# JackAILab/ConsistentID

Hardware: AMD Instinct MI355X
Metric: 512x512 SD1.5 images/sec/node @50 DDIM steps (higher is better)
Workload: dtype f16; 1 GPU; sd15 ConsistentID 512x512, 50 DDIM steps, batch 4/GPU (global 4), CFG batch 8, LoRA rank 128 merged, start_merge_step 30, hipGraph on; global_batch=4, parallelism=dp1 (images sharded, no in-step collective)

## Files before the change

### consistentid_amd/csrc/gemm.hip

```cpp
#include "xattn_core.h"
#include "gemm_args.h"
#include "../../include/cid.h"
#include <stdlib.h>

#ifndef CID_HALO_STAGGER
#define CID_HALO_STAGGER 1
#endif
#ifdef CID_CONV_TRACE
__device__ unsigned long long g_conv_trace[2 * 4096];
#define CONV_STAMP(k) do { if (tr_on) tr_ts[k] = __builtin_readcyclecounter(); } while (0)
#define CONV_FLUSH() do { if (tr_on && lane == 0 && tr_n + 8 <= 4096) { for (int q_ = 0; q_ < 8; ++q_) g_conv_trace[tr_slot * 4096 + tr_n + q_] = tr_ts[q_]; } tr_n += 8; } while (0)
#else
#define CONV_STAMP(k) do { } while (0)
#define CONV_FLUSH() do { } while (0)
#endif
#if defined(CID_GEMM_ABLATION)
#define CID_ABL(bit) ((a.ablate & (bit)) != 0)
#else
#define CID_ABL(bit) false
#endif

namespace {
using cidg::GemmArgs;
using cidg::wait_vmcnt;
// ... 936 lines not shown
                          : launch_one_ln<TM, TN, WM, WN, false, false, false, 3>(a, ncols, s);
    }
    return a.ln_s ? launch_one_ln<TM, TN, WM, WN, VMODE, true>(a, ncols, s) : launch_one_ln<TM, TN, WM, WN, VMODE, false>(a, ncols, s);
}

template <int TM, int TN, int WM, int WN, int ATT_D>
int launch_att(GemmArgs a, hipStream_t s) {
    a.n_begin = 0; a.n_end = a.N;
    return a.ln_s ? launch_one_ln<TM, TN, WM, WN, false, true, false, 2, ATT_D>(a, a.N, s)
                  : launch_one_ln<TM, TN, WM, WN, false, false, false, 2, ATT_D>(a, a.N, s);
}

template <int TM, int TN, int WM, int WN>
int launch_act(GemmArgs a, hipStream_t s) {
    a.n_begin = 0; a.n_end = a.N;
    return launch_one_ln<TM, TN, WM, WN, false, false, false, 2, 0, true>(a, a.N, s);
}

template <int TM, int TN, int WM, int WN>
int launch_halo(GemmArgs a, hipStream_t s) {
    constexpr int BM = 16 * TM * WM, BN = 16 * TN * WN, NW = WM * WN;
    constexpr int SMEM = 2 * (7 * NW * 1024) + 2 * (((BN / 8 + NW - 1) / NW) * NW * 1024);
    static_assert(SMEM <= 160 * 1024, "LDS budget");
    auto kern = igemm_halo_kernel<TM, TN, WM, WN>;
    static bool configured = false;
    if (!configured) {
        hipError_t herr = hipFuncSetAttribute((const void*)kern, hipFuncAttributeMaxDynamicSharedMemorySize, SMEM);
        if (herr != hipSuccess) {
            cid_set_error("cid_gemm_f16: cannot reserve %d bytes of LDS (%s)", SMEM, hipGetErrorString(herr));
            return -5;
        }
        configured = true;
    }
    a.n_begin = 0; a.n_end = a.N;
    dim3 grid((a.N + BN - 1) / BN, (a.M + BM - 1) / BM, a.splitk);
    a.xcd_pn = cidg::choose_xcd_pn((int)grid.x, (int)grid.y, 2.0 * a.N * a.ktot, (double)a.bytes_x1 + a.bytes_x2);
    hipLaunchKernelGGL(kern, grid, dim3(64 * NW), SMEM, s, a);
    if (a.splitk > 1) {
        const long items = (long)a.M * (a.N >> 2);
        const int g = (int)((items + 255) / 256 > 2048 ? 2048 : (items + 255) / 256);
        hipLaunchKernelGGL(splitk_epilogue_kernel, dim3(g), dim3(256), 0, s, a);
    }
    return 0;
}

template <int TM, int TN, int WM, int WN>
int launch(GemmArgs a, hipStream_t s) {
    const int n_plain = (a.mode == 2) ? a.n_vt0 : a.N;
    a.n_begin = 0; a.n_end = n_plain;
    int rc = launch_one<TM, TN, WM, WN, false>(a, n_plain, s);
    if (rc) return rc;
    if (a.splitk > 1) {
        const long items = (long)a.M * (a.N >> 2);
        const int grid = (int)((items + 255) / 256 > 2048 ? 2048 : (items + 255) / 256);
        hipLaunchKernelGGL(splitk_epilogue_kernel, dim3(grid), dim3(256), 0, s, a);
    }
    if (a.mode == 2 && a.N > a.n_vt0) {
        GemmArgs v = a;
        v.n_begin = a.n_vt0; v.n_end = a.N; v.splitk = 1;
        rc = launch_one<TM, TN, WM, WN, true>(v, a.N - a.n_vt0, s);
    }
    return rc;
}

}

int cidg::choose_xcd_pn(int gx, int gy, double w_bytes, double x_bytes) {
    static int on = -1;
    if (on < 0) { const char* e = getenv("CID_XCD_2D"); on = e ? atoi(e) : 1; }
    if (!on || ((long)gx * gy) % 8 != 0) return 0;
    int best = 0;
    double cost = 0.0;
    for (int pn = 1; pn <= 8; pn *= 2) {
        const int pm = 8 / pn;
        if (gx % pn != 0 || gy % pm != 0) continue;
        const double c = pm * w_bytes + pn * x_bytes;
        if (best == 0 || c < cost) { best = pn; cost = c; }
    }
    return best;
}

enum TileCfg { A256x160, B128x160, C64x160, G256x128, G128x128, O64x64, O128x32 };

static int plan_gemm(const cid_gemm_desc* d, GemmArgs& a, TileCfg& cfg, bool& halo, int& bm_out, bool& h32, bool& g32) {
    h32 = false;
    g32 = false;
    CID_CHECK_ARG(d && d->x1 && d->w && d->out, "cid_gemm_f16: null pointer");
    CID_CHECK_ARG(d->taps == 1 || d->taps == 9, "cid_gemm_f16: taps must be 1 or 9 (got %d)", d->taps);
    CID_CHECK_ARG(d->c1 > 0 && d->c1 % 32 == 0 && d->c2 >= 0 && d->c2 % 32 == 0 && (d->c1 + d->c2) % 64 == 0 &&
                  (d->c2 == 0 || d->c1 % 64 == 0),
                  "cid_gemm_f16: channel counts must be multiples of 64 (c1=%d c2=%d)", d->c1, d->c2);
    CID_CHECK_ARG(d->c2 == 0 || d->x2, "cid_gemm_f16: c2 > 0 needs x2");
    CID_CHECK_ARG(d->N > 0 && d->N % 32 == 0 && d->M > 0, "cid_gemm_f16: bad M/N (%d, %d)", d->M, d->N);
    CID_CHECK_ARG(d->mode >= 0 && d->mode <= 3, "cid_gemm_f16: bad mode %d", d->mode);
    CID_CHECK_ARG(d->ld1 % 8 == 0 && d->ldo % 8 == 0 && (d->c2 == 0 || d->ld2 % 8 == 0) && (!d->res || d->ldr % 8 == 0),
                  "cid_gemm_f16: row pitches (ld1, ld2, ldo, ldr) must keep 16-byte alignment");
    CID_CHECK_ARG((((uintptr_t)d->out | (uintptr_t)d->res | (uintptr_t)d->out2) & 15) == 0,
                  "cid_gemm_f16: out / out2 / res must be 16-byte aligned (rows are stored and the residual is read in 16-byte chunks)");
    CID_CHECK_ARG((d->ln_s == nullptr) == (d->ln_b == nullptr), "cid_gemm_f16: ln_s and ln_b come together");
    CID_CHECK_ARG(!d->ln_s || (d->taps == 1 && d->c2 == 0 && !d->bias && d->ln_eps > 0.f),
                  "cid_gemm_f16: the LayerNorm fold applies to one-source linears; the bias belongs in ln_b");
    a.x1 = (const half_t*)d->x1; a.x2 = (const half_t*)d->x2;
    a.c1 = d->c1; a.c2 = d->c2; a.ld1 = d->ld1; a.ld2 = d->ld2;
    a.w = (const half_t*)d->w; a.out = (half_t*)d->out; a.ldo = d->ldo;
    a.out2 = (half_t*)d->out2;
    CID_CHECK_ARG(!d->out2 || d->mode == 0, "cid_gemm_f16: out2 (a second destination) goes with the plain epilogue, mode 0");
    a.bias = (const half_t*)d->bias;
    a.rowbias = (const half_t*)d->rowbias; a.ld_rowbias = d->ld_rowbias;
    a.rows_per_sample = d->rows_per_sample > 0 ? d->rows_per_sample : 1;
    a.res = (const half_t*)d->res; a.ldr = d->ldr;
    a.M = d->M; a.N = d->N; a.taps = d->taps;
    a.Hi = d->Hi; a.Wi = d->Wi; a.Ho = d->Ho; a.Wo = d->Wo; a.stride = d->stride; a.up = d->up;
    a.mode = d->mode;
    a.vt = (half_t*)d->vt; a.n_vt0 = d->n_vt0; a.heads = d->heads; a.dhead = d->dhead;
    a.dvp = d->dvp; a.ntok = d->ntok;
    a.cslabs = (d->c1 + d->c2) / BK;
    a.ktot = d->taps * (d->c1 + d->c2);
    a.nslab = a.ktot / BK;
    a.splitk = 1;
    a.nloop = 1;
    a.nbuf = 2;
    a.xcd_pn = 0;
    a.att_kp = (const half_t*)d->att_kp; a.att_vp = (const half_t*)d->att_vp; a.att_kvrow = (const int*)d->att_kvrow;
    a.att_n_txt = d->att_n_txt; a.att_n_ip = d->att_n_ip; a.att_scale = d->att_ip_scale;
    a.att_krow = a.att_vrow = 0;
    a.ws = (float*)d->ws;
    a.ln_s = d->ln_s; a.ln_b = d->ln_b; a.ln_eps = d->ln_eps;
    a.gn_stats = d->gn_stats; a.gn_unit = d->N / 32;
    {
#if defined(CID_GEMM_ABLATION)
        static int ablate = -1;
        if (ablate < 0) { const char* e = getenv("CID_GEMM_ABLATE"); ablate = e ? atoi(e) : 0; }
        a.ablate = ablate;
#else
        a.ablate = 0;
#endif
    }
    {
        const long rows_in = (d->taps == 9) ? (long)(d->M / (d->Ho * d->Wo)) * d->Hi * d->Wi : (long)d->M;
        const long b1 = ((rows_in - 1) * d->ld1 + d->c1) * 2, b2 = d->c2 ? ((rows_in - 1) * d->ld2 + d->c2) * 2 : 0;
        const long bw = (long)d->N * a.ktot * 2;
        CID_CHECK_ARG(b1 < 0x7fffffffL && b2 < 0x7fffffffL && bw < 0x7fffffffL, "cid_gemm_f16: tensor exceeds 2 GiB");
        a.bytes_x1 = (unsigned)b1; a.bytes_x2 = (unsigned)b2; a.bytes_w = (unsigned)bw;
    }
    a.n_begin = 0; a.n_end = a.N;
    if (d->taps == 9) {
        CID_CHECK_ARG(d->Hi > 0 && d->Wi > 0 && d->Ho > 0 && d->Wo > 0 && (d->stride == 1 || d->stride == 2)
                      && (d->up == 0 || d->up == 1), "cid_gemm_f16: bad conv geometry");
        CID_CHECK_ARG(d->M % (d->Ho * d->Wo) == 0, "cid_gemm_f16: M is not batch * Ho * Wo");
    }
    CID_CHECK_ARG(d->pad_mode == 0 || d->pad_mode == 1, "cid_gemm_f16: bad pad_mode %d", d->pad_mode);
    CID_CHECK_ARG(d->pad_mode == 0 || (d->mode == 0 && d->taps == 9 && d->stride == 2 && d->up == 0 && d->Hi % 2 == 0 &&
                                       d->Wi % 2 == 0 && d->Ho == d->Hi / 2 && d->Wo == d->Wi / 2),
                  "cid_gemm_f16: pad_mode 1 needs mode 0, taps 9, stride 2, up 0, even Hi / Wi, Ho = Hi / 2 and Wo = Wi / 2 "
                  "(got mode %d taps %d stride %d up %d, %d x %d -> %d x %d)", d->mode, d->taps, d->stride, d->up, d->Hi, d->Wi,
                  d->Ho, d->Wo);
    a.tap0 = d->pad_mode == 1 ? 0 : -1;
    CID_CHECK_ARG(d->act == 0 || d->act == 1, "cid_gemm_f16: bad act %d", d->act);
    CID_CHECK_ARG(d->act == 0 || (d->mode == 0 && !d->gn_stats && !d->ws && !d->ln_s),
                  "cid_gemm_f16: act 1 needs mode 0 and no gn_stats / ws / ln_s (got mode %d)", d->mode);

    if (d->mode == 3) {
        CID_CHECK_ARG(d->att_kp && d->att_vp && d->att_kvrow, "cid_gemm_f16: mode 3 needs att_kp / att_vp / att_kvrow");
        CID_CHECK_ARG(d->taps == 1 && d->c2 == 0 && !d->bias && !d->rowbias && !d->res && !d->gn_stats,
                      "cid_gemm_f16: mode 3 is a plain projection (no bias / residual / statistics)");
        CID_CHECK_ARG(d->heads > 0 && d->dhead > 0 && d->N == d->heads * d->dhead && (d->dhead == 64 || d->dhead == 80 || d->dhead == 160),
                      "cid_gemm_f16: mode 3 needs N = heads * dhead with dhead in {64, 80, 160} (got %d x %d, N = %d)", d->heads, d->dhead, d->N);
        CID_CHECK_ARG(d->att_n_txt == 77 && d->att_n_ip == 4, "cid_gemm_f16: mode 3 is built for the reference's 77 + 4 context (got %d + %d)",
                      d->att_n_txt, d->att_n_ip);
        CID_CHECK_ARG(d->ntok > 0 && d->M % d->ntok == 0 && d->ntok % 64 == 0, "cid_gemm_f16: mode 3 needs ntok (tokens per sample, a multiple of 64)");
        const int qks = (d->dhead + 15) / 16, dvt = (d->dhead + 31) / 32;
        a.att_krow = (long)d->heads * 3 * qks * 512;
        a.att_vrow = (long)d->heads * dvt * 6 * 512;
        if (d->dhead == 64) { cfg = G128x128; bm_out = 128; CID_CHECK_ARG(d->N % 128 == 0 && d->ntok % 128 == 0, "cid_gemm_f16: mode 3, dhead 64: N and ntok multiples of 128"); }
        else {
            CID_CHECK_ARG(d->N % 160 == 0, "cid_gemm_f16: mode 3, dhead %d: N = %d is not a multiple of the 160-channel tile", d->dhead, d->N);
            if (d->ntok % 128 == 0 && (long)(d->M / 128) * (d->N / 160) >= 256) { cfg = B128x160; bm_out = 128; }
            else { cfg = C64x160; bm_out = 64; }
        }
        halo = false;
        return 0;
    }
    const int n_plain = (d->mode == 2) ? d->n_vt0 : d->N;
    const long target = 2048;
    auto waves = [&](int bm_, int bn_, int w) {
        return (long)((a.M + bm_ - 1) / bm_) * ((n_plain + bn_ - 1) / bn_) * w;
    };
    int bm = 0, bn = 0, nw = 0;
    bool small_tiles = (d->mode == 1) && (a.nslab <= 10 || waves(256, 128, 1) < 1024);
    if (d->mode == 1) {
        static int g_tile = -1;
        if (g_tile < 0) { const char* e = getenv("CID_GEGLU_TILE"); g_tile = e ? atoi(e) : 0; }
        if (g_tile == 1) small_tiles = false;
        if (g_tile == 2) small_tiles = true;
        if (d->N % 128 != 0) { cfg = O64x64; bm = 64; bn = 64; nw = 4; }
        else if (waves(256, 128, 8) >= target && !small_tiles) { cfg = G256x128; bm = 256; bn = 128; nw = 8; }
        else { cfg = G128x128; bm = 128; bn = 128; nw = 8; }
    } else if (n_plain % 160 == 0) {
        static int f_tile = -1, f_sk = -1;
        if (f_tile < 0) { const char* e = getenv("CID_GEMM_TILE"); f_tile = e ? atoi(e) : 0; }
        if (f_sk < 0) { const char* e = getenv("CID_GEMM_SK"); f_sk = e ? atoi(e) : 0; }
        const bool can_split = (d->mode == 0) && a.ws != nullptr && !a.ln_s;
        auto tiles = [&](int bm_) { return (long)((a.M + bm_ - 1) / bm_) * (n_plain / 160); };
        auto sk_for = [&](int bm_) {
            long t = tiles(bm_);
            int sk = (int)((256 + t - 1) / t);
            if (!can_split) sk = 1;
            if (sk > 16) sk = 16;
            while (sk > 1 && a.nslab / sk < 6) --sk;
            while (sk > 1 && (int64_t)sk * a.M * a.N * 4 > d->ws_bytes) --sk;
            return sk;
        };
        int pick = 0;
        bool nosplit = false;
        static int prefer128 = -1;
        if (prefer128 < 0) { const char* e = getenv("CID_GEMM_PREFER128"); prefer128 = e ? atoi(e) : 1; }
        if (f_tile) pick = f_tile;
        else if (d->taps == 1 && tiles(256) >= 256) {
            pick = (prefer128 || (d->mode == 2 && tiles(256) <= 512 && tiles(128) >= 512)) ? 2 : 1;
            nosplit = true;
        } else if (d->taps == 1 && tiles(128) >= 256 && (a.nslab <= 40 || prefer128)) { pick = 2; nosplit = true; }
        else if (d->taps == 1 && tiles(64) >= 256 && a.nslab <= 20) { pick = 3; nosplit = true; }
        else if (tiles(256) * sk_for(256) >= 256) pick = 1;
        else if (tiles(128) * sk_for(128) >= 256) pick = 2;
        else pick = 3;
        if (pick == 1)      { cfg = A256x160; bm = 256; bn = 160; nw = 8; }
// ... 9 lines not shown
    if (d->mode == 1) CID_CHECK_ARG(d->N % 64 == 0, "cid_gemm_f16: GEGLU needs N %% 64 == 0");
    if (d->mode == 1 && (cfg == G128x128 || cfg == G256x128) && d->taps == 1 && d->c2 == 0 && a.M % bm == 0) {
        static int f_nl = -1;
        if (f_nl < 0) { const char* e = getenv("CID_GEGLU_NLOOP"); f_nl = e ? atoi(e) : 0; }
        const int nt = d->N / bn;
        const long tiles = (long)(a.M / bm) * nt;
        int nl = f_nl > 0 ? f_nl : (int)(tiles / (cfg == G128x128 ? 512 : 256));
        if (nl > nt) nl = nt;
        while (nl > 1 && nt % nl != 0) --nl;
        if (nl > 1 && (long)nl * bn * a.ktot * 2 < 0x7fffffffL) a.nloop = nl;
    }
    if (d->mode == 1 && d->taps == 1 && d->c2 == 0 && !a.ln_s && d->N % 160 == 0 && a.M % 256 == 0 && a.cslabs >= 16) {
        static int f_g32 = -1;
        if (f_g32 < 0) { const char* e = getenv("CID_GEGLU_H32"); f_g32 = e ? atoi(e) : 1; }
        const int nt = d->N / 160;
        const long tiles = (long)(a.M / 256) * nt;
        int nl = (int)(tiles / 256);
        if (nl > nt) nl = nt;
        while (nl > 1 && nt % nl != 0) --nl;
        if (f_g32 && tiles >= 256 && nl >= 1 && (long)nl * 160 * a.ktot * 2 < 0x7fffffffL) {
            g32 = true;
            a.nloop = nl;
            bm = 256;
        }
    }
    if (d->mode == 2) {
        CID_CHECK_ARG(d->vt && d->ntok % 16 == 0 && d->M % d->ntok == 0 && d->n_vt0 % bn == 0 && d->dhead > 0
                      && d->heads > 0 && d->dvp >= d->dhead && (d->N - d->n_vt0) % 16 == 0,
                      "cid_gemm_f16: bad QKV/V^T description");
    }
    if (d->mode == 0 && a.ws && !a.ln_s && a.nslab >= 16 && n_plain % 160 != 0) {
        const long w = waves(bm, bn, nw);
        if (w < target) {
            int sk = (int)((target + w - 1) / w);
            if (sk > 8) sk = 8;
            while (sk > 1 && a.nslab / sk < 8) --sk;
            while (sk > 1 && (int64_t)sk * a.M * a.N * 4 > d->ws_bytes) --sk;
            a.splitk = sk;
        }
    }
    {
        static int f_nb = -1;
        if (f_nb < 0) { const char* e = getenv("CID_GEMM_NBUF"); f_nb = e ? atoi(e) : 0; }
        const bool legal = (cfg == A256x160 || cfg == B128x160 || cfg == C64x160) && d->mode != 1 && !d->act;
        const long wgs = (long)((a.M + bm - 1) / bm) * ((n_plain + bn - 1) / bn) * a.splitk;
        const bool want = cfg == A256x160 ? (a.nslab / a.splitk >= 4) : (wgs <= 256 && a.nslab / a.splitk >= 8);
        if (legal && (f_nb == 3 || (f_nb == 0 && want))) a.nbuf = 3;
    }
    static int no_halo = -1;
    if (no_halo < 0) { const char* e = getenv("CID_GEMM_NOHALO"); no_halo = e ? atoi(e) : 0; }
    halo = false;
    if (cfg == A256x160 && !no_halo && !d->act && d->mode == 0 && d->taps == 9 && d->stride == 1 && d->up == 0 && d->Wo == d->Wi &&
        d->Ho == d->Hi) {
        const int HW = d->Ho * d->Wo;
        const int seg = 256 < HW ? 256 : HW;
        const bool rows_ok = (seg % d->Wo == 0) && (HW % seg == 0) && (256 % seg == 0) && (d->M % 256 == 0);
        const int nh = (256 / seg) * (seg / d->Wo + 2) * (d->Wo + 2);
        if (rows_ok && nh <= 448) {
            halo = true;
            if (a.splitk > a.cslabs) a.splitk = a.cslabs;
        }
    }
    {
        static int no_h32 = -1;
        static int only256 = 0;
        if (no_h32 < 0) { const char* e = getenv("CID_CONV_H32"); no_h32 = (e && atoi(e) == 0) ? 1 : 0; only256 = (e && atoi(e) == 2) ? 1 : 0; }
        const int HW = d->taps == 9 ? d->Ho * d->Wo : 0;
        const bool shape_ok = !no_h32 && !d->act && d->mode == 0 && d->taps == 9 && d->stride == 1 && (d->up == 0 || d->up == 1) &&
                              d->Wo == (d->Wi << d->up) && d->Ho == (d->Hi << d->up) && d->N % 160 == 0 && HW >= 64 &&
                              (!d->rowbias || (a.rows_per_sample >= 64 && a.rows_per_sample % 64 == 0));
        for (int bm_try = 256; shape_ok && !h32 && bm_try >= (only256 ? 256 : 128); bm_try >>= 1) {
            const int seg = bm_try < HW ? bm_try : HW;
            if (seg % d->Wo != 0 || HW % seg != 0 || bm_try % seg != 0 || d->M % bm_try != 0) continue;
            if (d->up && (seg != bm_try || (seg / d->Wo) % 2 != 0)) continue;
            const int nh = (bm_try / seg) * (((seg / d->Wo) >> d->up) + 2) * ((d->Wo >> d->up) + 2);
            if (nh > 400) continue;
            const long tiles = (long)(d->M / bm_try) * (d->N / 160);
            if (tiles < 256 || (bm_try == 128 && a.cslabs > 10)) continue;
            h32 = true; halo = false;
            bm = bm_try;
            a.splitk = 1;
        }
    }
    bm_out = bm;
    if (a.gn_stats) {
        const bool ok = d->mode == 0 && a.splitk == 1 && (cfg == A256x160 || cfg == B128x160 || cfg == C64x160) &&
                        d->N % 32 == 0 && 80 % a.gn_unit == 0 && d->M % bm == 0;
        CID_CHECK_ARG(ok, "cid_gemm_f16: gn_stats requested for a launch that cannot emit them (ask cid_gemm_stats_rows first)");
    }
    return 0;
}

extern "C" int cid_gemm_stats_rows(const cid_gemm_desc* d) {
    if (!d) return 0;
    cid_gemm_desc q = *d;
    q.gn_stats = nullptr;
    GemmArgs a;
    TileCfg cfg;
    bool halo, h32, g32;
    int bm = 0;
    if (plan_gemm(&q, a, cfg, halo, bm, h32, g32) != 0) return 0;
    const int unit = d->N / 32;
    const bool ok = d->mode == 0 && d->act == 0 && a.splitk == 1 && (cfg == A256x160 || cfg == B128x160 || cfg == C64x160) &&
                    d->N % 32 == 0 && unit > 0 && 80 % unit == 0 && d->M % bm == 0;
    return ok ? bm : 0;
}

extern "C" int cid_gemm_f16(const cid_gemm_desc* d, cid_stream_t stream) {
    GemmArgs a;
    TileCfg cfg;
    bool halo, h32, g32;
    int bm = 0;
    int rc = plan_gemm(d, a, cfg, halo, bm, h32, g32);
    if (rc) return rc;
    hipStream_t s = (hipStream_t)stream;
    if (g32) {
        a.n_begin = 0; a.n_end = a.N;
        rc = cidg::launch_geglu_h32(a, s);
        if (rc) return rc;
        CID_CHECK_LAUNCH("cid_gemm_f16");
        return 0;
    }
    if (a.mode == 3) {
        if (cfg == G128x128) rc = launch_att<2, 4, 4, 2, 64>(a, s);
        else if (cfg == B128x160) rc = a.dhead == 80 ? launch_att<2, 5, 4, 2, 80>(a, s) : launch_att<2, 5, 4, 2, 160>(a, s);
        else rc = a.dhead == 80 ? launch_att<2, 5, 2, 2, 80>(a, s) : launch_att<2, 5, 2, 2, 160>(a, s);
        if (rc) return rc;
        CID_CHECK_LAUNCH("cid_gemm_f16");
        return 0;
    }
    if (d->act) {
        switch (cfg) {
            case A256x160: rc = launch_act<4, 5, 4, 2>(a, s); break;
            case B128x160: rc = launch_act<2, 5, 4, 2>(a, s); break;
            case C64x160:  rc = launch_act<2, 5, 2, 2>(a, s); break;
            case G256x128: rc = launch_act<4, 4, 4, 2>(a, s); break;
            case G128x128: rc = launch_act<2, 4, 4, 2>(a, s); break;
            case O64x64:   rc = launch_act<2, 2, 2, 2>(a, s); break;
            case O128x32:  rc = launch_act<2, 2, 4, 1>(a, s); break;
        }
        if (rc) return rc;
        CID_CHECK_LAUNCH("cid_gemm_f16");
        return 0;
    }
    if (h32) {
        a.n_begin = 0; a.n_end = a.N;
        rc = cidg::launch_conv_h32(a, bm, s);
        if (rc) return rc;
        CID_CHECK_LAUNCH("cid_gemm_f16");
        return 0;
    }
    if (halo) {
        rc = launch_halo<4, 5, 4, 2>(a, s);
        if (rc) return rc;
        CID_CHECK_LAUNCH("cid_gemm_f16");
        return 0;
    }
    switch (cfg) {
        case A256x160: rc = launch<4, 5, 4, 2>(a, s); break;
        case B128x160: rc = launch<2, 5, 4, 2>(a, s); break;
        case C64x160:  rc = launch<2, 5, 2, 2>(a, s); break;
        case G256x128: rc = launch<4, 4, 4, 2>(a, s); break;
        case G128x128: rc = launch<2, 4, 4, 2>(a, s); break;
        case O64x64:   rc = launch<2, 2, 2, 2>(a, s); break;
        case O128x32:  rc = launch<2, 2, 4, 1>(a, s); break;
    }
    if (rc) return rc;
    CID_CHECK_LAUNCH("cid_gemm_f16");
    return 0;
}
```

### consistentid_amd/csrc/gemm_args.h

```cpp
#pragma once
#include "common.h"

namespace cidg {

struct GemmArgs {
    const half_t* x1; const half_t* x2;
    int c1, c2, ld1, ld2;
    const half_t* w;
    half_t* out; int ldo;
    half_t* out2;
    const half_t* bias;
    const half_t* rowbias; int ld_rowbias; int rows_per_sample;
    const half_t* res; int ldr;
    int M, N, taps;
    int Hi, Wi, Ho, Wo, stride, up;
    int mode;
    half_t* vt; int n_vt0, heads, dhead, dvp, ntok;
    int n_begin, n_end;
    int ktot;
    int nslab;
    int cslabs;
    int splitk;
    int nloop;
    int nbuf;
    const half_t* att_kp; const half_t* att_vp; const int* att_kvrow;
    long att_krow, att_vrow;
    int att_n_txt, att_n_ip;
    float att_scale;
    unsigned bytes_x1, bytes_x2, bytes_w;
    float* ws;
    const float* ln_s;
    const float* ln_b;
    float ln_eps;
    float* gn_stats;
    int gn_unit;
    int ablate;
    int xcd_pn;
    int tap0;
};

CID_DEVINL void xcd_tile(const GemmArgs& a, int& nb, int& mb) {
    const int gx = gridDim.x, gy = gridDim.y;
    int bid = blockIdx.y * gx + blockIdx.x;
    if (a.xcd_pn > 0) {
        const int pn = a.xcd_pn;
        const int x = bid & 7, l = bid >> 3;
        const int bnc = gx / pn;
        nb = (x % pn) * bnc + l % bnc;
        mb = (x / pn) * (gy * pn >> 3) + l / bnc;
    } else {
        const int nwg = gx * gy;
        if ((nwg & 7) == 0) bid = (bid & 7) * (nwg >> 3) + (bid >> 3);
        nb = bid % gx;
        mb = bid / gx;
    }
}

int choose_xcd_pn(int gx, int gy, double w_bytes, double x_bytes);

CID_DEVINL void wait_vmcnt(int n) {
#define CID_VM(N) case N: asm volatile("s_waitcnt vmcnt(" #N ")" ::: "memory"); break;
    switch (n) {
        CID_VM(0) CID_VM(1) CID_VM(2) CID_VM(3) CID_VM(4) CID_VM(5) CID_VM(6) CID_VM(7) CID_VM(8) CID_VM(9)
        CID_VM(10) CID_VM(11) CID_VM(12) CID_VM(13) CID_VM(14) CID_VM(15) CID_VM(16) CID_VM(17) CID_VM(18)
        CID_VM(19) CID_VM(20) CID_VM(21) CID_VM(22) CID_VM(23) CID_VM(24) CID_VM(25) CID_VM(26) CID_VM(27)
        CID_VM(28) CID_VM(29) CID_VM(30) CID_VM(31) CID_VM(32)
        default: asm volatile("s_waitcnt vmcnt(0)" ::: "memory"); break;
    }
#undef CID_VM
}

int launch_conv_h32(const GemmArgs& a, int bm, hipStream_t s);

int launch_geglu_h32(const GemmArgs& a, hipStream_t s);

}
```

### consistentid_amd/csrc/linear_h32.hip

```cpp
#include "gemm_args.h"
#include "../../include/cid.h"

namespace {
using cidg::GemmArgs;
using cidg::wait_vmcnt;

constexpr int BN = 160, BK = 64;
constexpr int WST = BN * 128;
constexpr int NSTG = 3;
constexpr int WQ = 5;
constexpr int BIAS_IMG = 512;

typedef __attribute__((address_space(3))) void lds_void;

CID_DEVINL int key(int r) { return (r >> 1) & 7; }

template <int TM>
__global__ void __launch_bounds__(512, 1)
geglu_h32_kernel(GemmArgs a) {
#if defined(__HIP_DEVICE_COMPILE__)
    constexpr int BM = 128 * TM;
    constexpr int XST = BM * 128;
    constexpr int STG = XST + WST;
    constexpr int XQ = BM / 32;
    extern __shared__ __attribute__((aligned(16))) char smem[];
    char* bias_img = smem + NSTG * STG;
    const int tid = threadIdx.x;
    const int lane = tid & 63;
    const int wave = __builtin_amdgcn_readfirstlane(tid >> 6);
    const int r8 = lane >> 3, c8 = lane & 7;
    const int l32 = lane & 31, lh = lane >> 5;
    int nb_, mb_;
    cidg::xcd_tile(a, nb_, mb_);
    const int ncs = a.cslabs, nloop = a.nloop;
    const int F = ncs * nloop;
    const int n0 = nb_ * BN * nloop;
    const int m0 = mb_ * BM;
    const bool is_loader = wave >= 4;
    const int lw = wave & 3;

    if (is_loader) {
        const __amdgpu_buffer_rsrc_t rs_x = __builtin_amdgcn_make_buffer_rsrc((void*)a.x1, 0, a.bytes_x1, 0x00020000);
        const __amdgpu_buffer_rsrc_t rs_w = __builtin_amdgcn_make_buffer_rsrc((void*)a.w, 0, a.bytes_w, 0x00020000);
        const __amdgpu_buffer_rsrc_t rs_b = __builtin_amdgcn_make_buffer_rsrc((void*)a.bias, 0, a.bias ? (unsigned)(a.N * 2) : 0u, 0x00020000);
        unsigned xoff[XQ], woff[WQ];
#pragma unroll
        for (int q = 0; q < XQ; ++q) {
            const int R = (lw + 4 * q) * 8 + r8;
            xoff[q] = (unsigned)(((long)(m0 + R) * a.ld1 + (c8 ^ key(R)) * 8) * 2);
        }
#pragma unroll
        for (int q = 0; q < WQ; ++q) {
            const int R = (lw + 4 * q) * 8 + r8;
            woff[q] = (unsigned)(((long)(n0 + R) * a.ktot + (c8 ^ key(R)) * 8) * 2);
        }
        const unsigned wstep = (unsigned)((long)BN * a.ktot * 2);
        int is_cs = 0, is_j = 0, is_st = 0;
        unsigned is_w = 0u;
        auto issue_next = [&]() -> int {
            int n = XQ + WQ;
            if (is_cs == 0 && lw == 0) {
                char* dst = bias_img + (is_j & 1) * BIAS_IMG;
                const unsigned boff = (unsigned)((n0 + is_j * BN) * 2 + lane * 4);
                __builtin_amdgcn_raw_ptr_buffer_load_lds(rs_b, (lds_void*)dst, 4, boff, 0, 0, 0);
                __builtin_amdgcn_raw_ptr_buffer_load_lds(rs_b, (lds_void*)(dst + 256), 4, boff + 256u, 0, 0, 0);
                n += 2;
            }
            char* xs = smem + is_st * STG;
            char* ws = xs + XST;
            const unsigned coff = (unsigned)(is_cs * BK * 2);
#pragma unroll
            for (int q = 0; q < XQ; ++q)
                __builtin_amdgcn_raw_ptr_buffer_load_lds(rs_x, (lds_void*)(xs + (lw + 4 * q) * 1024), 16, xoff[q], coff, 0, 0);
#pragma unroll
            for (int q = 0; q < WQ; ++q)
                __builtin_amdgcn_raw_ptr_buffer_load_lds(rs_w, (lds_void*)(ws + (lw + 4 * q) * 1024), 16, woff[q], coff + is_w, 0, 0);
            if (++is_cs == ncs) { is_cs = 0; ++is_j; is_w += wstep; }
            is_st = is_st + 1 == NSTG ? 0 : is_st + 1;
            return n;
        };
        issue_next();
        const int n1 = F > 1 ? issue_next() : 0;
        wait_vmcnt(n1);
        __builtin_amdgcn_s_barrier();
        for (int f = 0; f < F; ++f) {
            const int n = f + 2 < F ? issue_next() : 0;
            wait_vmcnt(n);
            __builtin_amdgcn_s_barrier();
        }
        asm volatile("s_waitcnt vmcnt(0)" ::: "memory");
    } else {
        int xaddr[TM];
#pragma unroll
        for (int t = 0; t < TM; ++t) {
            const int row = (lw * TM + t) * 32 + l32;
            xaddr[t] = row * 128 + ((lh ^ key(row)) << 4);
        }
        const int wlane = XST + l32 * 128 + ((lh ^ key(l32)) << 4);
        f32x16 acc[TM][5];
#pragma unroll
        for (int t = 0; t < TM; ++t)
#pragma unroll
            for (int c = 0; c < 5; ++c)
#pragma unroll
                for (int i = 0; i < 16; ++i) acc[t][c][i] = 0.f;
        auto read_frags = [&](const char* stg, int j, half8 (&xf)[TM], half8 (&wf)[5]) {
#pragma unroll
            for (int t = 0; t < TM; ++t) xf[t] = *reinterpret_cast<const half8*>(stg + (xaddr[t] ^ (j << 5)));
            const char* wsb = stg + (wlane ^ (j << 5));
#pragma unroll
            for (int c = 0; c < 5; ++c) wf[c] = *reinterpret_cast<const half8*>(wsb + c * 4096);
        };
        auto mma = [&](const half8 (&xf)[TM], const half8 (&wf)[5]) {
#pragma unroll
            for (int t = 0; t < TM; ++t)
#pragma unroll
                for (int c = 0; c < 5; ++c) acc[t][c] = mfma32(wf[c], xf[t], acc[t][c]);
        };
        auto interleave = [&]() {
            if constexpr (TM == 2) {
#pragma unroll
                for (int i = 0; i < 7; ++i) {
                    __builtin_amdgcn_sched_group_barrier(0x8, 1, 0);
                    __builtin_amdgcn_sched_group_barrier(0x100, 1, 0);
                }
                __builtin_amdgcn_sched_group_barrier(0x8, 3, 0);
            } else {
                __builtin_amdgcn_sched_group_barrier(0x100, 1, 0);
#pragma unroll
                for (int i = 0; i < 5; ++i) {
                    __builtin_amdgcn_sched_group_barrier(0x8, 1, 0);
                    __builtin_amdgcn_sched_group_barrier(0x100, 1, 0);
                }
            }
        };
        __builtin_amdgcn_s_barrier();
        half8 xf0[TM], wf0[5], xf1[TM], wf1[5];
        read_frags(smem, 0, xf0, wf0);
        int cs = 0, jt = 0, st = 0;
        for (int f = 0; f < F; ++f) {
            const char* stg = smem + st * STG;
            const int stn = st + 1 == NSTG ? 0 : st + 1;
            read_frags(stg, 1, xf1, wf1);
            mma(xf0, wf0);
            interleave();
            __builtin_amdgcn_sched_barrier(0);
            read_frags(stg, 2, xf0, wf0);
            mma(xf1, wf1);
            interleave();
            __builtin_amdgcn_sched_barrier(0);
            read_frags(stg, 3, xf1, wf1);
            mma(xf0, wf0);
            interleave();
            __builtin_amdgcn_sched_barrier(0);
            asm volatile("s_waitcnt lgkmcnt(0)" ::: "memory");
            __builtin_amdgcn_s_barrier();
            __builtin_amdgcn_sched_barrier(0);
            read_frags(smem + stn * STG, 0, xf0, wf0);
            mma(xf1, wf1);
            interleave();
            __builtin_amdgcn_sched_barrier(0);
            st = stn;
            if (++cs == ncs) {
                const half_t* bimg = reinterpret_cast<const half_t*>(bias_img + (jt & 1) * BIAS_IMG);
                const bool has_bias = a.bias != nullptr;
                const int ocol = ((n0 + jt * BN) >> 1) + 8 * lh;
#pragma unroll
                for (int t = 0; t < TM; ++t) {
                    half_t* orow = a.out + (long)(m0 + (lw * TM + t) * 32 + l32) * a.ldo + ocol;
#pragma unroll
                    for (int c = 0; c < 5; ++c) {
                        unsigned pk[2][2];
#pragma unroll
                        for (int g = 0; g < 2; ++g) {
                            float bv[4] = {0.f, 0.f, 0.f, 0.f}, bg[4] = {0.f, 0.f, 0.f, 0.f};
                            if (has_bias) {
                                const half4 hv = *reinterpret_cast<const half4*>(bimg + c * 32 + 8 * g + 4 * lh);
                                const half4 hg = *reinterpret_cast<const half4*>(bimg + c * 32 + 16 + 8 * g + 4 * lh);
#pragma unroll
                                for (int i = 0; i < 4; ++i) { bv[i] = (float)hv[i]; bg[i] = (float)hg[i]; }
                            }
                            float o[4];
#pragma unroll
                            for (int i = 0; i < 4; ++i)
                                o[i] = (acc[t][c][4 * g + i] + bv[i]) * gelu_erf_f(acc[t][c][4 * (g + 2) + i] + bg[i]);
                            const half2v p0 = {(half_t)o[0], (half_t)o[1]}, p1 = {(half_t)o[2], (half_t)o[3]};
                            pk[g][0] = __builtin_bit_cast(unsigned, p0);
                            pk[g][1] = __builtin_bit_cast(unsigned, p1);
                        }
                        typedef unsigned u32x2 __attribute__((ext_vector_type(2)));
                        typedef unsigned u32x4 __attribute__((ext_vector_type(4)));
                        const u32x2 s0 = __builtin_amdgcn_permlane32_swap(pk[0][0], pk[1][0], false, false);
                        const u32x2 s1 = __builtin_amdgcn_permlane32_swap(pk[0][1], pk[1][1], false, false);
                        const u32x4 v = {s0[0], s1[0], s0[1], s1[1]};
                        *reinterpret_cast<u32x4*>(orow + c * 16) = v;
#pragma unroll
                        for (int i = 0; i < 16; ++i) acc[t][c][i] = 0.f;
                    }
                }
                cs = 0; ++jt;
                __builtin_amdgcn_sched_barrier(0);
            }
        }
    }
#endif
}

}

template <int TM>
static int launch_geglu_tm(const GemmArgs& a, hipStream_t s) {
    constexpr int BM = 128 * TM;
    constexpr int SMEM = NSTG * (BM * 128 + WST) + 2 * BIAS_IMG;
    static_assert(SMEM <= 160 * 1024, "LDS budget");
    CID_CHECK_ARG(a.cslabs >= 3, "cid_gemm_f16: the linear_h32 GEGLU launch needs >= 3 channel slabs (got %d)", a.cslabs);
    static bool configured = false;
    if (!configured) {
        hipError_t herr = hipFuncSetAttribute((const void*)geglu_h32_kernel<TM>, hipFuncAttributeMaxDynamicSharedMemorySize, SMEM);
        if (herr != hipSuccess) {
            cid_set_error("cid_gemm_f16: cannot reserve %d bytes of LDS (%s)", SMEM, hipGetErrorString(herr));
            return -5;
        }
        configured = true;
    }
    dim3 grid(a.N / BN / a.nloop, a.M / BM, 1);
    GemmArgs b = a;
    b.xcd_pn = cidg::choose_xcd_pn((int)grid.x, (int)grid.y, 2.0 * a.N * a.ktot, (double)a.bytes_x1);
    hipLaunchKernelGGL(geglu_h32_kernel<TM>, grid, dim3(512), SMEM, s, b);
    return 0;
}

int cidg::launch_geglu_h32(const GemmArgs& a, hipStream_t s) { return launch_geglu_tm<2>(a, s); }
```

Measured before the change: 7.631 images/s.

## Route plain 1x1 linears through the h32 GEMM kernel with residual and GroupNorm-stats epilogue

Generalizes the GEGLU-only linear_h32 kernel into a template over tile height, pipeline depth and epilogue type. Adds plain and plain-with-GroupNorm-statistics epilogues that fuse bias, residual add, dual output stores and per-unit sum/sum-of-squares reduction. Plain one-source linears with N divisible by 160 are routed to it by default, with a 4-stage pipeline at 128-row tiles. This aims to replace the older tile configurations for these linears with the faster pipelined kernel, at the cost of added complexity and more LDS use for the statistics scratch.

```diff
diff --git a/consistentid_amd/csrc/gemm.hip b/consistentid_amd/csrc/gemm.hip
--- a/consistentid_amd/csrc/gemm.hip
+++ b/consistentid_amd/csrc/gemm.hip
@@ -1042,9 +1042,18 @@
 
 enum TileCfg { A256x160, B128x160, C64x160, G256x128, G128x128, O64x64, O128x32 };
 
-static int plan_gemm(const cid_gemm_desc* d, GemmArgs& a, TileCfg& cfg, bool& halo, int& bm_out, bool& h32, bool& g32) {
+static int plain_h32_tile(int M, int N, int cslabs) {
+    const long nt = N / 160;
+    if (M % 256 == 0 && (long)(M / 256) * nt >= 256 && cslabs >= 16) return 256;
+    const long t128 = (long)(M / 128) * nt;
+    if (M % 128 == 0 && (t128 >= 256 || (t128 >= 128 && cslabs <= 40))) return 128;
+    return 0;
+}
+
+static int plan_gemm(const cid_gemm_desc* d, GemmArgs& a, TileCfg& cfg, bool& halo, int& bm_out, bool& h32, bool& g32, bool& p32) {
     h32 = false;
     g32 = false;
+    p32 = false;
     CID_CHECK_ARG(d && d->x1 && d->w && d->out, "cid_gemm_f16: null pointer");
     CID_CHECK_ARG(d->taps == 1 || d->taps == 9, "cid_gemm_f16: taps must be 1 or 9 (got %d)", d->taps);
     CID_CHECK_ARG(d->c1 > 0 && d->c1 % 32 == 0 && d->c2 >= 0 && d->c2 % 32 == 0 && (d->c1 + d->c2) % 64 == 0 &&
@@ -1102,6 +1111,7 @@
         const long bw = (long)d->N * a.ktot * 2;
         CID_CHECK_ARG(b1 < 0x7fffffffL && b2 < 0x7fffffffL && bw < 0x7fffffffL, "cid_gemm_f16: tensor exceeds 2 GiB");
         a.bytes_x1 = (unsigned)b1; a.bytes_x2 = (unsigned)b2; a.bytes_w = (unsigned)bw;
+        a.bytes_res = a.bytes_out = 0u;
     }
     a.n_begin = 0; a.n_end = a.N;
     if (d->taps == 9) {
@@ -1277,9 +1287,36 @@
             a.splitk = 1;
         }
     }
+    if (d->mode == 0 && d->taps == 1 && d->c2 == 0 && !d->rowbias && !d->act && !a.ln_s && d->N % 160 == 0 && d->N >= 320 &&
+        a.cslabs >= 4) {
+        static int f_p32 = -1;
+        if (f_p32 < 0) { const char* e = getenv("CID_PLAIN_H32"); f_p32 = e ? atoi(e) : 1; }
+        int pbm = 0;
+        if (f_p32 == 256 || f_p32 == 128) pbm = f_p32;
+        else if (f_p32) pbm = plain_h32_tile(a.M, d->N, a.cslabs);
+        if (pbm && a.M % pbm == 0) {
+            const int nt = d->N / 160;
+            const long tiles = (long)(a.M / pbm) * nt;
+            int nl = (int)(tiles / 256);
+            if (nl < 1) nl = 1;
+            if (nl > nt) nl = nt;
+            while (nl > 1 && nt % nl != 0) --nl;
+            const long br = d->res ? ((long)(a.M - 1) * d->ldr + d->N) * 2 : 0;
+            const long bo = ((long)(a.M - 1) * d->ldo + d->N) * 2;
+            if ((long)nl * 160 * a.ktot * 2 < 0x7fffffffL && br < 0x7fffffffL && bo < 0x7fffffffL) {
+                p32 = true;
+                a.bytes_res = (unsigned)br;
+                a.bytes_out = (unsigned)bo;
+                a.nloop = nl;
+                a.splitk = 1;
+                a.nbuf = 2;
+                bm = pbm;
+            }
+        }
+    }
     bm_out = bm;
     if (a.gn_stats) {
-        const bool ok = d->mode == 0 && a.splitk == 1 && (cfg == A256x160 || cfg == B128x160 || cfg == C64x160) &&
+        const bool ok = d->mode == 0 && a.splitk == 1 && (p32 || cfg == A256x160 || cfg == B128x160 || cfg == C64x160) &&
                         d->N % 32 == 0 && 80 % a.gn_unit == 0 && d->M % bm == 0;
         CID_CHECK_ARG(ok, "cid_gemm_f16: gn_stats requested for a launch that cannot emit them (ask cid_gemm_stats_rows first)");
     }
@@ -1292,11 +1329,11 @@
     q.gn_stats = nullptr;
     GemmArgs a;
     TileCfg cfg;
-    bool halo, h32, g32;
+    bool halo, h32, g32, p32;
     int bm = 0;
-    if (plan_gemm(&q, a, cfg, halo, bm, h32, g32) != 0) return 0;
+    if (plan_gemm(&q, a, cfg, halo, bm, h32, g32, p32) != 0) return 0;
     const int unit = d->N / 32;
-    const bool ok = d->mode == 0 && d->act == 0 && a.splitk == 1 && (cfg == A256x160 || cfg == B128x160 || cfg == C64x160) &&
+    const bool ok = d->mode == 0 && d->act == 0 && a.splitk == 1 && (p32 || cfg == A256x160 || cfg == B128x160 || cfg == C64x160) &&
                     d->N % 32 == 0 && unit > 0 && 80 % unit == 0 && d->M % bm == 0;
     return ok ? bm : 0;
 }
@@ -1304,11 +1341,18 @@
 extern "C" int cid_gemm_f16(const cid_gemm_desc* d, cid_stream_t stream) {
     GemmArgs a;
     TileCfg cfg;
-    bool halo, h32, g32;
+    bool halo, h32, g32, p32;
     int bm = 0;
-    int rc = plan_gemm(d, a, cfg, halo, bm, h32, g32);
+    int rc = plan_gemm(d, a, cfg, halo, bm, h32, g32, p32);
     if (rc) return rc;
     hipStream_t s = (hipStream_t)stream;
+    if (p32) {
+        a.n_begin = 0; a.n_end = a.N;
+        rc = cidg::launch_plain_h32(a, bm, s);
+        if (rc) return rc;
+        CID_CHECK_LAUNCH("cid_gemm_f16");
+        return 0;
+    }
     if (g32) {
         a.n_begin = 0; a.n_end = a.N;
         rc = cidg::launch_geglu_h32(a, s);
diff --git a/consistentid_amd/csrc/gemm_args.h b/consistentid_amd/csrc/gemm_args.h
--- a/consistentid_amd/csrc/gemm_args.h
+++ b/consistentid_amd/csrc/gemm_args.h
@@ -28,6 +28,7 @@
     int att_n_txt, att_n_ip;
     float att_scale;
     unsigned bytes_x1, bytes_x2, bytes_w;
+    unsigned bytes_res, bytes_out;
     float* ws;
     const float* ln_s;
     const float* ln_b;
@@ -74,4 +75,6 @@
 
 int launch_geglu_h32(const GemmArgs& a, hipStream_t s);
 
+int launch_plain_h32(const GemmArgs& a, int bm, hipStream_t s);
+
 }
diff --git a/consistentid_amd/csrc/linear_h32.hip b/consistentid_amd/csrc/linear_h32.hip
--- a/consistentid_amd/csrc/linear_h32.hip
+++ b/consistentid_amd/csrc/linear_h32.hip
@@ -7,17 +7,30 @@
 
 constexpr int BN = 160, BK = 64;
 constexpr int WST = BN * 128;
-constexpr int NSTG = 3;
 constexpr int WQ = 5;
 constexpr int BIAS_IMG = 512;
+constexpr int EPI_GEGLU = 0, EPI_PLAIN = 1, EPI_PLAIN_GN = 2;
+constexpr int GN_COL = 640;
+constexpr int GN_UNITS = 128;
+constexpr int lds_bytes(int tm, int ns, int epi) {
+    return ns * (tm * 128 * 128 + WST) + 2 * BIAS_IMG + (epi == EPI_PLAIN_GN ? 4 * (GN_COL + GN_UNITS) : 0);
+}
 
 typedef __attribute__((address_space(3))) void lds_void;
 
 CID_DEVINL int key(int r) { return (r >> 1) & 7; }
 
-template <int TM>
+CID_DEVINL float half_sum(float v) {
+#define CID_DPP_ADD(CTRL, ROWS) v += __builtin_bit_cast(float, __builtin_amdgcn_update_dpp(0, __builtin_bit_cast(int, v), CTRL, ROWS, 0xf, false))
+    CID_DPP_ADD(0x128, 0xf); CID_DPP_ADD(0x124, 0xf); CID_DPP_ADD(0x122, 0xf); CID_DPP_ADD(0x121, 0xf);
+    CID_DPP_ADD(0x142, 0xa);
+#undef CID_DPP_ADD
+    return v;
+}
+
+template <int TM, int NSTG, int EPI>
 __global__ void __launch_bounds__(512, 1)
-geglu_h32_kernel(GemmArgs a) {
+linear_h32_kernel(GemmArgs a) {
 #if defined(__HIP_DEVICE_COMPILE__)
     constexpr int BM = 128 * TM;
     constexpr int XST = BM * 128;
@@ -25,6 +38,8 @@
     constexpr int XQ = BM / 32;
     extern __shared__ __attribute__((aligned(16))) char smem[];
     char* bias_img = smem + NSTG * STG;
+    char* gn_col = bias_img + 2 * BIAS_IMG;
+    char* gn_units = gn_col + 4 * GN_COL;
     const int tid = threadIdx.x;
     const int lane = tid & 63;
     const int wave = __builtin_amdgcn_readfirstlane(tid >> 6);
@@ -79,15 +94,24 @@
             is_st = is_st + 1 == NSTG ? 0 : is_st + 1;
             return n;
         };
-        issue_next();
-        const int n1 = F > 1 ? issue_next() : 0;
-        wait_vmcnt(n1);
+        int hist[NSTG - 1];
+#pragma unroll
+        for (int k = 0; k < NSTG - 1; ++k) hist[k] = k < F ? issue_next() : 0;
+        auto flying = [&]() { int n = 0;
+#pragma unroll
+            for (int k = 1; k < NSTG - 1; ++k) n += hist[k];
+            return n; };
+        wait_vmcnt(flying());
         __builtin_amdgcn_s_barrier();
         for (int f = 0; f < F; ++f) {
-            const int n = f + 2 < F ? issue_next() : 0;
-            wait_vmcnt(n);
+            const int n = f + NSTG - 1 < F ? issue_next() : 0;
+#pragma unroll
+            for (int k = 0; k + 1 < NSTG - 1; ++k) hist[k] = hist[k + 1];
+            hist[NSTG - 2] = n;
+            wait_vmcnt(flying());
             __builtin_amdgcn_s_barrier();
         }
+        if constexpr (EPI == EPI_PLAIN_GN) __builtin_amdgcn_s_barrier();
         asm volatile("s_waitcnt vmcnt(0)" ::: "memory");
     } else {
         int xaddr[TM];
@@ -134,10 +158,44 @@
                 }
             }
         };
+        const bool has_res = EPI != EPI_GEGLU && a.res != nullptr;
+        const __amdgpu_buffer_rsrc_t rs_r = __builtin_amdgcn_make_buffer_rsrc((void*)a.res, 0, has_res ? a.bytes_res : 0u, 0x00020000);
+        const __amdgpu_buffer_rsrc_t rs_o = __builtin_amdgcn_make_buffer_rsrc((void*)a.out, 0, EPI != EPI_GEGLU ? a.bytes_out : 0u, 0x00020000);
+        const __amdgpu_buffer_rsrc_t rs_o2 = __builtin_amdgcn_make_buffer_rsrc((void*)a.out2, 0, EPI != EPI_GEGLU && a.out2 ? a.bytes_out : 0u, 0x00020000);
+        unsigned roff[TM], ooff[TM];
+        half8 rcur[TM][2];
+#pragma unroll
+        for (int t = 0; t < TM; ++t) {
+            roff[t] = (unsigned)(((long)(m0 + (lw * TM + t) * 32 + l32) * a.ldr + n0 + 8 * lh) * 2);
+            ooff[t] = (unsigned)(((long)(m0 + (lw * TM + t) * 32 + l32) * a.ldo + n0 + 8 * lh) * 2);
+        }
+        int jt = 0;
+        auto load_res = [&](half8 (&r)[TM][2], int c) {
+            const unsigned soff = (unsigned)((jt * BN + c * 32) * 2);
+#pragma unroll
+            for (int t = 0; t < TM; ++t)
+#pragma unroll
+                for (int p = 0; p < 2; ++p)
+                    r[t][p] = __builtin_bit_cast(half8, __builtin_amdgcn_raw_buffer_load_b128(rs_r, roff[t] + (unsigned)(p * 32), soff, 0));
+        };
+        int fold_jt = -1;
+        auto fold_stats = [&](int j) {
+            const int nu = BN / a.gn_unit;
+            if (lw == 0 && lane < nu) {
+                double S = 0.0, Q = 0.0;
+#pragma unroll
+                for (int w_ = 0; w_ < 4; ++w_) {
+                    const float* up = reinterpret_cast<const float*>(gn_units + w_ * GN_UNITS) + 2 * lane;
+                    S += (double)up[0]; Q += (double)up[1];
+                }
+                float* dst = a.gn_stats + ((long)(m0 / BM) * (a.N / a.gn_unit) + (n0 + j * BN) / a.gn_unit + lane) * 2;
+                dst[0] = (float)S; dst[1] = (float)Q;
+            }
+        };
         __builtin_amdgcn_s_barrier();
         half8 xf0[TM], wf0[5], xf1[TM], wf1[5];
         read_frags(smem, 0, xf0, wf0);
-        int cs = 0, jt = 0, st = 0;
+        int cs = 0, st = 0;
         for (int f = 0; f < F; ++f) {
             const char* stg = smem + st * STG;
             const int stn = st + 1 == NSTG ? 0 : st + 1;
@@ -156,67 +214,186 @@
             asm volatile("s_waitcnt lgkmcnt(0)" ::: "memory");
             __builtin_amdgcn_s_barrier();
             __builtin_amdgcn_sched_barrier(0);
+            if constexpr (EPI == EPI_PLAIN_GN) {
+                if (fold_jt >= 0) { fold_stats(fold_jt); fold_jt = -1; }
+            }
+            if constexpr (EPI != EPI_GEGLU && TM == 1) {
+                if (cs + 1 == ncs) load_res(rcur, 0);
+                __builtin_amdgcn_sched_barrier(0);
+            }
             read_frags(smem + stn * STG, 0, xf0, wf0);
             mma(xf1, wf1);
             interleave();
             __builtin_amdgcn_sched_barrier(0);
             st = stn;
             if (++cs == ncs) {
-                const half_t* bimg = reinterpret_cast<const half_t*>(bias_img + (jt & 1) * BIAS_IMG);
-                const bool has_bias = a.bias != nullptr;
-                const int ocol = ((n0 + jt * BN) >> 1) + 8 * lh;
-#pragma unroll
-                for (int t = 0; t < TM; ++t) {
-                    half_t* orow = a.out + (long)(m0 + (lw * TM + t) * 32 + l32) * a.ldo + ocol;
+                if constexpr (EPI == EPI_GEGLU) {
+                    const half_t* bimg = reinterpret_cast<const half_t*>(bias_img + (jt & 1) * BIAS_IMG);
+                    const bool has_bias = a.bias != nullptr;
+                    const int ocol = ((n0 + jt * BN) >> 1) + 8 * lh;
+#pragma unroll
+                    for (int t = 0; t < TM; ++t) {
+                        half_t* orow = a.out + (long)(m0 + (lw * TM + t) * 32 + l32) * a.ldo + ocol;
+#pragma unroll
+                        for (int c = 0; c < 5; ++c) {
+                            unsigned pk[2][2];
+#pragma unroll
+                            for (int g = 0; g < 2; ++g) {
+                                float bv[4] = {0.f, 0.f, 0.f, 0.f}, bg[4] = {0.f, 0.f, 0.f, 0.f};
+                                if (has_bias) {
+                                    const half4 hv = *reinterpret_cast<const half4*>(bimg + c * 32 + 8 * g + 4 * lh);
+                                    const half4 hg = *reinterpret_cast<const half4*>(bimg + c * 32 + 16 + 8 * g + 4 * lh);
+#pragma unroll
+                                    for (int i = 0; i < 4; ++i) { bv[i] = (float)hv[i]; bg[i] = (float)hg[i]; }
+                                }
+                                float o[4];
+#pragma unroll
+                                for (int i = 0; i < 4; ++i)
+                                    o[i] = (acc[t][c][4 * g + i] + bv[i]) * gelu_erf_f(acc[t][c][4 * (g + 2) + i] + bg[i]);
+                                const half2v p0 = {(half_t)o[0], (half_t)o[1]}, p1 = {(half_t)o[2], (half_t)o[3]};
+                                pk[g][0] = __builtin_bit_cast(unsigned, p0);
+                                pk[g][1] = __builtin_bit_cast(unsigned, p1);
+                            }
+                            typedef unsigned u32x2 __attribute__((ext_vector_type(2)));
+                            typedef unsigned u32x4 __attribute__((ext_vector_type(4)));
+                            const u32x2 s0 = __builtin_amdgcn_permlane32_swap(pk[0][0], pk[1][0], false, false);
+                            const u32x2 s1 = __builtin_amdgcn_permlane32_swap(pk[0][1], pk[1][1], false, false);
+                            const u32x4 v = {s0[0], s1[0], s0[1], s1[1]};
+                            *reinterpret_cast<u32x4*>(orow + c * 16) = v;
+#pragma unroll
+                            for (int i = 0; i < 16; ++i) acc[t][c][i] = 0.f;
+                        }
+                    }
+                } else {
+                    const half_t* bimg = reinterpret_cast<const half_t*>(bias_img + (jt & 1) * BIAS_IMG) + 8 * lh;
+                    const bool has_bias = a.bias != nullptr;
+                    float sq[5][2][8];
+                    float* colw = reinterpret_cast<float*>(gn_col + lw * GN_COL);
 #pragma unroll
                     for (int c = 0; c < 5; ++c) {
-                        unsigned pk[2][2];
-#pragma unroll
-                        for (int g = 0; g < 2; ++g) {
-                            float bv[4] = {0.f, 0.f, 0.f, 0.f}, bg[4] = {0.f, 0.f, 0.f, 0.f};
-                            if (has_bias) {
-                                const half4 hv = *reinterpret_cast<const half4*>(bimg + c * 32 + 8 * g + 4 * lh);
-                                const half4 hg = *reinterpret_cast<const half4*>(bimg + c * 32 + 16 + 8 * g + 4 * lh);
-#pragma unroll
-                                for (int i = 0; i < 4; ++i) { bv[i] = (float)hv[i]; bg[i] = (float)hg[i]; }
+                        half8 rn[TM][2];
+                        if (TM != 1 && c == 0) load_res(rcur, 0);
+                        if (c + 1 < 5) load_res(rn, c + 1);
+                        float gs[2][8], gq[2][8];
+#pragma unroll
+                        for (int p = 0; p < 2; ++p)
+#pragma unroll
+                            for (int k = 0; k < 8; ++k) { gs[p][k] = 0.f; gq[p][k] = 0.f; }
+#pragma unroll
+                        for (int t = 0; t < TM; ++t) {
+#pragma unroll
+                            for (int p = 0; p < 2; ++p) {
+                                float v[8];
+#pragma unroll
+                                for (int i = 0; i < 4; ++i) {
+                                    typedef unsigned u32x2 __attribute__((ext_vector_type(2)));
+                                    const float lo = acc[t][c][8 * p + i], hi = acc[t][c][8 * p + 4 + i];
+                                    const u32x2 sw = __builtin_amdgcn_permlane32_swap(__builtin_bit_cast(unsigned, lo), __builtin_bit_cast(unsigned, hi), false, false);
+                                    const unsigned s0 = sw[0], s1 = sw[1];
+                                    v[i] = __builtin_bit_cast(float, s0);
+                                    v[4 + i] = __builtin_bit_cast(float, s1);
+                                }
+                                typedef unsigned u32x4 __attribute__((ext_vector_type(4)));
+                                u32x4 bu = *reinterpret_cast<const u32x4*>(bimg + c * 32 + p * 16);
+#pragma unroll
+                                for (int k = 0; k < 4; ++k) bu[k] = has_bias ? bu[k] : 0u;
+                                const half8 b = __builtin_bit_cast(half8, bu);
+#pragma unroll
+                                for (int k = 0; k < 8; ++k) v[k] = (v[k] + (float)b[k]) + (float)rcur[t][p][k];
+                                half8 o;
+#pragma unroll
+                                for (int k = 0; k < 8; ++k) o[k] = (half_t)v[k];
+                                const unsigned soff = (unsigned)((jt * BN + c * 32) * 2);
+                                __builtin_amdgcn_raw_buffer_store_b128(__builtin_bit_cast(u32x4, o), rs_o, ooff[t] + (unsigned)(p * 32), soff, 0);
+                                __builtin_amdgcn_raw_buffer_store_b128(__builtin_bit_cast(u32x4, o), rs_o2, ooff[t] + (unsigned)(p * 32), soff, 0);
+                                if constexpr (EPI == EPI_PLAIN_GN) {
+#pragma unroll
+                                    for (int k = 0; k < 8; ++k) { const float f = (float)o[k]; gs[p][k] += f; gq[p][k] = __builtin_fmaf(f, f, gq[p][k]); }
+                                }
                             }
-                            float o[4];
-#pragma unroll
-                            for (int i = 0; i < 4; ++i)
-                                o[i] = (acc[t][c][4 * g + i] + bv[i]) * gelu_erf_f(acc[t][c][4 * (g + 2) + i] + bg[i]);
-                            const half2v p0 = {(half_t)o[0], (half_t)o[1]}, p1 = {(half_t)o[2], (half_t)o[3]};
-                            pk[g][0] = __builtin_bit_cast(unsigned, p0);
-                            pk[g][1] = __builtin_bit_cast(unsigned, p1);
-                        }
-                        typedef unsigned u32x2 __attribute__((ext_vector_type(2)));
-                        typedef unsigned u32x4 __attribute__((ext_vector_type(4)));
-                        const u32x2 s0 = __builtin_amdgcn_permlane32_swap(pk[0][0], pk[1][0], false, false);
-                        const u32x2 s1 = __builtin_amdgcn_permlane32_swap(pk[0][1], pk[1][1], false, false);
-                        const u32x4 v = {s0[0], s1[0], s0[1], s1[1]};
-                        *reinterpret_cast<u32x4*>(orow + c * 16) = v;
-#pragma unroll
-                        for (int i = 0; i < 16; ++i) acc[t][c][i] = 0.f;
+#pragma unroll
+                            for (int i = 0; i < 16; ++i) acc[t][c][i] = 0.f;
+                        }
+                        if (c + 1 < 5) {
+#pragma unroll
+                            for (int t = 0; t < TM; ++t)
+#pragma unroll
+                                for (int p = 0; p < 2; ++p) rcur[t][p] = rn[t][p];
+                        }
+                        if constexpr (EPI == EPI_PLAIN_GN) {
+#pragma unroll
+                            for (int p = 0; p < 2; ++p)
+#pragma unroll
+                                for (int k = 0; k < 8; ++k) { gs[p][k] = half_sum(gs[p][k]); sq[c][p][k] = half_sum(gq[p][k]); }
+                            if (l32 == 16) {
+#pragma unroll
+                                for (int p = 0; p < 2; ++p)
+#pragma unroll
+                                    for (int h = 0; h < 2; ++h) {
+                                        const f32x4 w4 = {gs[p][4 * h], gs[p][4 * h + 1], gs[p][4 * h + 2], gs[p][4 * h + 3]};
+                                        *reinterpret_cast<f32x4*>(colw + c * 32 + p * 16 + 8 * lh + 4 * h) = w4;
+                                    }
+                            }
+                        }
+                    }
+                    if constexpr (EPI == EPI_PLAIN_GN) {
+                        const int nu = BN / a.gn_unit;
+                        auto unit_total = [&]() {
+                            asm volatile("s_waitcnt lgkmcnt(0)" ::: "memory");
+                            double tot = 0.0;
+                            if (lane < nu)
+                                for (int k = 0; k < a.gn_unit; ++k) tot += (double)colw[lane * a.gn_unit + k];
+                            asm volatile("s_waitcnt lgkmcnt(0)" ::: "memory");
+                            return (float)tot;
+                        };
+                        const float S = unit_total();
+                        if (l32 == 16) {
+#pragma unroll
+                            for (int c = 0; c < 5; ++c)
+#pragma unroll
+                                for (int p = 0; p < 2; ++p)
+#pragma unroll
+                                    for (int h = 0; h < 2; ++h) {
+                                        const f32x4 w4 = {sq[c][p][4 * h], sq[c][p][4 * h + 1], sq[c][p][4 * h + 2], sq[c][p][4 * h + 3]};
+                                        *reinterpret_cast<f32x4*>(colw + c * 32 + p * 16 + 8 * lh + 4 * h) = w4;
+                                    }
+                        }
+                        const float Q = unit_total();
+                        if (lane < nu) {
+                            float* up = reinterpret_cast<float*>(gn_units + lw * GN_UNITS) + 2 * lane;
+                            up[0] = S; up[1] = Q;
+                        }
+                        asm volatile("s_waitcnt lgkmcnt(0)" ::: "memory");
+                        fold_jt = jt;
                     }
                 }
                 cs = 0; ++jt;
                 __builtin_amdgcn_sched_barrier(0);
             }
         }
+        if constexpr (EPI == EPI_PLAIN_GN) {
+            __builtin_amdgcn_s_barrier();
+            fold_stats(fold_jt);
+        }
     }
 #endif
 }
 
 }
 
-template <int TM>
-static int launch_geglu_tm(const GemmArgs& a, hipStream_t s) {
+template <int TM, int NSTG, int EPI>
+static int launch_h32(const GemmArgs& a, hipStream_t s) {
     constexpr int BM = 128 * TM;
-    constexpr int SMEM = NSTG * (BM * 128 + WST) + 2 * BIAS_IMG;
+    constexpr int SMEM = lds_bytes(TM, NSTG, EPI);
     static_assert(SMEM <= 160 * 1024, "LDS budget");
-    CID_CHECK_ARG(a.cslabs >= 3, "cid_gemm_f16: the linear_h32 GEGLU launch needs >= 3 channel slabs (got %d)", a.cslabs);
+    CID_CHECK_ARG(a.cslabs >= NSTG, "cid_gemm_f16: this linear_h32 launch needs >= %d channel slabs (got %d)", NSTG, a.cslabs);
+    CID_CHECK_ARG(a.M % BM == 0 && a.N % (BN * a.nloop) == 0, "cid_gemm_f16: linear_h32 takes whole %d x %d tiles (M=%d N=%d nloop=%d)",
+                  BM, BN, a.M, a.N, a.nloop);
+    if constexpr (EPI == EPI_PLAIN_GN)
+        CID_CHECK_ARG(a.gn_unit >= 10 && BN % a.gn_unit == 0, "cid_gemm_f16: linear_h32 statistics units of %d channels", a.gn_unit);
     static bool configured = false;
     if (!configured) {
-        hipError_t herr = hipFuncSetAttribute((const void*)geglu_h32_kernel<TM>, hipFuncAttributeMaxDynamicSharedMemorySize, SMEM);
+        hipError_t herr = hipFuncSetAttribute((const void*)linear_h32_kernel<TM, NSTG, EPI>, hipFuncAttributeMaxDynamicSharedMemorySize, SMEM);
         if (herr != hipSuccess) {
             cid_set_error("cid_gemm_f16: cannot reserve %d bytes of LDS (%s)", SMEM, hipGetErrorString(herr));
             return -5;
@@ -226,8 +403,13 @@
     dim3 grid(a.N / BN / a.nloop, a.M / BM, 1);
     GemmArgs b = a;
     b.xcd_pn = cidg::choose_xcd_pn((int)grid.x, (int)grid.y, 2.0 * a.N * a.ktot, (double)a.bytes_x1);
-    hipLaunchKernelGGL(geglu_h32_kernel<TM>, grid, dim3(512), SMEM, s, b);
+    hipLaunchKernelGGL((linear_h32_kernel<TM, NSTG, EPI>), grid, dim3(512), SMEM, s, b);
     return 0;
 }
 
-int cidg::launch_geglu_h32(const GemmArgs& a, hipStream_t s) { return launch_geglu_tm<2>(a, s); }
+int cidg::launch_geglu_h32(const GemmArgs& a, hipStream_t s) { return launch_h32<2, 3, EPI_GEGLU>(a, s); }
+
+int cidg::launch_plain_h32(const GemmArgs& a, int bm, hipStream_t s) {
+    if (bm == 256) return a.gn_stats ? launch_h32<2, 3, EPI_PLAIN_GN>(a, s) : launch_h32<2, 3, EPI_PLAIN>(a, s);
+    return a.gn_stats ? launch_h32<1, 4, EPI_PLAIN_GN>(a, s) : launch_h32<1, 4, EPI_PLAIN>(a, s);
+}
```

Result: no change. 7.689 images/s (median of 6 runs) (+0.8%).
